# Triton-AI/Triton-Racer-Sim

Measured on AMD Instinct MI355X. Metric: env-steps/s (whole node) at N envs x 120x160 RGB, higher is better.
Workload: dtype f32 state / f64 nearest-point / u8 image; 1 GPU; 1024 envs/GPU x 1 GPU, bicycle physics + L1 nearest point + 120x160 RGB pinhole rasteriser = BASELINE configs[2], generated_track 1185 pts, synthetic controls seed 0x5EED, auto-reset; envs_total=1024, envs_per_gpu=1024, img_h=120, img_w=160, depth=False, steps_per_launch=1, step_mode=resident worker (posted steps), prewarm_steps=8400, launcher=self

## Files before the change

triton-racer-sim_amd/csrc/trsim_device.hpp:

```cpp
#pragma once
#include <hip/hip_runtime.h>

#include <cstdint>

#include "../../include/trsim.h"
#include "../../include/trsim_spec.h"
#include "trsim_plan.hpp"
#include "trsim_tables.hpp"

#ifndef TRS_ABLATE
#define TRS_ABLATE 0
#endif

namespace trsim {

struct PParams {
    float *x, *y, *z, *yaw, *v, *speed, *cte, *ep_return, *last_return, *steer_filt;
    int32_t *seg_idx, *ep_len;
    uint8_t *done, *pending;
    const float *ctl_steer, *ctl_thr, *ctl_brk;
    const uint8_t* ctl_reset;
    int ctl_stride;
    float4* cam;
    const unsigned char* blob;
    const float* start_yaw;
    const float* tangent_g;
    unsigned long long* stats;
    unsigned long long* fault;
    int n_envs, env_id_base, envs_per_wg, np;
    int off_py, off_pz, off_tan, blob_bytes, off_scratch, tan_in_lds;
    int off_gstart, off_gpts, grid_nx, grid_nz;
    double grid_x0, grid_z0;
    float map_x0f, map_z0f, inv_cellf;
    float dt, max_steer, inv_wheelbase, accel_max, drag_lin, roll_res, brake_max;
    float v_max, v_rev_max, offtrack_cte, offtrack_penalty, cam_fwd;
    int auto_reset, synth, n_steps, write_cam;
// ... 265 lines not shown
    best_out = __hiloint2double(__builtin_amdgcn_readlane(__double2hiint(best), 63), __builtin_amdgcn_readlane(__double2loint(best), 63));
}

__device__ __forceinline__ NearParams near_of(const PParams& p)
{
    return NearParams{p.np, p.off_py, p.off_pz, p.off_gstart, p.off_gpts, p.grid_nx, p.grid_nz, p.grid_x0, p.grid_z0};
}

struct EnvRegs {
    float x, y, z, yaw, v, sf, epr, speed, cte;
    int seg, epl, done, pend;
};

__device__ __forceinline__ void env_load(const PParams& p, int e, EnvRegs& s)
{
    s.pend = coherent_load(&p.pending[e]); s.done = coherent_load(&p.done[e]);
    s.sf = coherent_load(&p.steer_filt[e]);
    s.x = coherent_load(&p.x[e]); s.y = coherent_load(&p.y[e]); s.z = coherent_load(&p.z[e]);
    s.yaw = coherent_load(&p.yaw[e]); s.v = coherent_load(&p.v[e]);
    s.seg = coherent_load(&p.seg_idx[e]);
    s.epr = coherent_load(&p.ep_return[e]);
    s.epl = coherent_load(&p.ep_len[e]);
    s.speed = 0.f; s.cte = 0.f;
}

__device__ __forceinline__ void env_store(const PParams& p, int e, const EnvRegs& s, int lane)
{
    if (lane == 0) {
        p.x[e] = s.x; p.y[e] = s.y; p.z[e] = s.z; p.yaw[e] = s.yaw; p.v[e] = s.v;
        p.speed[e] = s.speed; p.cte[e] = s.cte; p.seg_idx[e] = s.seg; p.done[e] = (uint8_t)s.done;
        p.ep_return[e] = s.epr; p.ep_len[e] = s.epl; p.steer_filt[e] = s.sf; p.pending[e] = (uint8_t)s.pend;
    }
}
struct StepOut { float4 cam; float pitch; int is_done, do_reset; };

template <bool WT, typename T>
__device__ __forceinline__ void store_out(T* ptr, T v)
{
    if constexpr (WT) __hip_atomic_store(ptr, v, __ATOMIC_RELAXED, __HIP_MEMORY_SCOPE_SYSTEM);
    else *ptr = v;
}

template <bool WT, bool STORE_LR = true, bool SEL = false>
__device__ __forceinline__ void env_advance(const PParams& p, const unsigned char* lphys, int e, EnvRegs& s, uint32_t t, int synth,
                                            float steer, float thr, float brk, uint8_t rin, int lane, StepOut& o, const trsim::HillBlock* hill = nullptr)
{
    const double* lpx = reinterpret_cast<const double*>(lphys);
    const double* lpy = reinterpret_cast<const double*>(lphys + p.off_py);
    const double* lpz = reinterpret_cast<const double*>(lphys + p.off_pz);
    const float2* ltan = reinterpret_cast<const float2*>(lphys + p.off_tan);
    const int gid = p.env_id_base + e;
    float sf = s.sf;
    const int prev_idx = s.seg;
    float epr = s.epr;
    int epl = s.epl;
    const int do_reset = (s.pend != 0) || (rin != 0) || (p.auto_reset && s.done != 0);
    float x1, y0, z1, yaw1, v2, hs, hc;
    if (do_reset) {
        const int si = (int)(((long long)TRS_START_STRIDE * gid) % p.np);
        x1 = (float)lpx[si]; y0 = (float)lpy[si]; z1 = (float)lpz[si];
        yaw1 = p.start_yaw[si]; v2 = 0.0f; sf = 0.0f;
        if constexpr (SEL) spec_sincos_sel(yaw1, hs, hc); else spec_sincos(yaw1, hs, hc);
    } else {
        if (synth) synth_controls(p.seed, (uint32_t)gid, t, sf, steer, thr);
        steer = clampf(steer, -1.0f, 1.0f);
        thr = clampf(thr, -1.0f, 1.0f);
        brk = clampf(brk, 0.0f, 1.0f);
// ... 67 lines not shown
        const size_t ci = (size_t)k * (size_t)p.ctl_stride + (size_t)e;
        steer = p.ctl_steer[ci]; thr = p.ctl_thr[ci]; brk = p.ctl_brk ? p.ctl_brk[ci] : 0.0f;
    }
    StepOut o;
    env_advance<false, true, SEL>(p, lphys, e, s, t, p.synth, steer, thr, brk, rin, lane, o, hill);
    if (lane == 0) {
        if (p.write_cam) cam_out[e] = o.cam;
        *lcam_slot = o.cam;
        if (hill) {
            if (p.write_cam) hill->cam_pitch[(size_t)(t & (kRing - 1)) * p.n_envs + e] = o.pitch;
            if (lpitch_slot) *lpitch_slot = o.pitch;
        }
        if (o.is_done) atomicAdd(&p.stats[0], 1ull);
        if (o.do_reset) atomicAdd(&p.stats[1], 1ull);
        __hip_atomic_store(pprog_j, k + 1, __ATOMIC_RELEASE, __HIP_MEMORY_SCOPE_WORKGROUP);
    }
}

__device__ __forceinline__ f2v ray_step(f2v kk2, f2v cns)
{
#ifdef TRS_PACKED_RAY_STEP
    return kk2 * cns;
#else
    float dx, dz;
    asm("v_mul_f32 %0, %1, %2" : "=v"(dx) : "v"(kk2.x), "v"(cns.x));
    asm("v_mul_f32 %0, %1, %2" : "=v"(dz) : "v"(kk2.y), "v"(cns.y));
    return f2v{dx, dz};
#endif
}

struct RasterThread {
    const f2v* lrow;
    const float* lrowdepth;
    unsigned pal_off;
    f2v ufa, ufb, ufc, ufd;
    unsigned gwm1, ghm1, pitch;
    int cg, vstart, vground, col_off, row_bytes;
};

__device__ __forceinline__ RasterThread raster_thread(const RParams& p, const unsigned char* lds, int tid)
{
    RasterThread t;
    t.lrow = reinterpret_cast<const f2v*>(lds + p.off_rowtab);
    t.lrowdepth = reinterpret_cast<const float*>(lds + p.off_depth);
    t.pal_off = (unsigned)p.off_pal;
    const float half_w = (float)(p.W / 2);
    t.gwm1 = (unsigned)(p.map_w - 1); t.ghm1 = (unsigned)(p.map_h - 1);
    t.cg = tid % p.gpr;
    const int r0 = tid / p.gpr;
    const float uf0 = (float)(t.cg << 2) + 0.5f - half_w;
    t.ufa = f2v{uf0, uf0}; t.ufb = f2v{uf0 + 1.0f, uf0 + 1.0f}; t.ufc = f2v{uf0 + 2.0f, uf0 + 2.0f}; t.ufd = f2v{uf0 + 3.0f, uf0 + 3.0f};
    t.pitch = (unsigned)p.map_pitch_b;
    t.vstart = r0 < p.rows_per_pass ? r0 : p.H;
    t.vground = t.vstart;
    while (t.vground < p.uni_rows) t.vground += p.rows_per_pass;
    t.row_bytes = p.gpr * 12;
    t.col_off = t.cg * 12;
    return t;
}

struct FrameDesc { __amdgpu_buffer_rsrc_t rgb, dep; };

template <bool DEPTH>
__device__ __forceinline__ FrameDesc frame_desc(const RParams& p, uint8_t* img, float* dep, int e)
{
    FrameDesc f;
    f.rgb = __builtin_amdgcn_make_buffer_rsrc(img + (size_t)e * ((size_t)p.gpe * 12), 0, (int)((size_t)p.gpe * 12), 0x00020000);
    f.dep = f.rgb;
    if constexpr (DEPTH) f.dep = __builtin_amdgcn_make_buffer_rsrc(dep + (size_t)e * ((size_t)p.gpe * 4), 0, (int)((size_t)p.gpe * 16), 0x00020000);
    return f;
}

template <bool DEPTH>
__device__ __forceinline__ void raster_uniform_rows(const RParams& p, const RasterThread& t, const FrameDesc& f, int uni_rows = -1)
{
    const int nu = uni_rows < 0 ? p.uni_rows : uni_rows;
    for (int v = t.vstart; v < nu; v += p.rows_per_pass) {
        const uint32_t c = *(lds_u32p)(uintptr_t)(t.pal_off + ((unsigned)v << 4));
        const u3v px3 = {__builtin_amdgcn_perm(c, c, 0x04020100u), __builtin_amdgcn_perm(c, c, 0x05040201u), __builtin_amdgcn_perm(c, c, 0x06050402u)};
        __builtin_amdgcn_raw_buffer_store_b96(px3, f.rgb, t.col_off + v * t.row_bytes, 0, TRS_STORE_AUX);
        if constexpr (DEPTH) {
            const unsigned dz = __float_as_uint(t.lrowdepth[v]);
            const u4v d4 = {dz, dz, dz, dz};
            __builtin_amdgcn_raw_buffer_store_b128(d4, f.dep, (t.cg + v * p.gpr) * 16, 0, TRS_STORE_AUX);
        }
    }
}

template <bool DEPTH, bool UNI_CHECK = false>
__device__ __forceinline__ void raster_ground_rows(const RParams& p, const RasterThread& t, const FrameDesc& f, const float4 cam)
{
    const f2v sc = {cam.z, cam.w}, cns = {cam.w, -cam.z}, camxz = {cam.x, cam.y};
    f2v rt = t.lrow[t.vground < p.H ? t.vground : 0];
    for (int v = t.vground; v < p.H; v += p.rows_per_pass) {
        const int vn = v + p.rows_per_pass;
        const f2v rtn = t.lrow[vn < p.H ? vn : v];
        const unsigned pal_a = t.pal_off + ((unsigned)v << 4);
        const f2v lz2 = {rt.x, rt.x}, kk2 = {rt.y, rt.y};
        f2v a;
        if constexpr (UNI_CHECK) {
            a.x = __builtin_fmaf(rt.x, sc.x, camxz.x);
            a.y = __builtin_fmaf(rt.x, sc.y, camxz.y);
        } else {
            a = __builtin_elementwise_fma(lz2, sc, camxz);
        }
        const f2v d = ray_step(kk2, cns);
        auto shade = [&](f2v uf) -> uint32_t {
            const f2v g = __builtin_elementwise_fma(uf, d, a);
            const unsigned ix = min(cvt_u32_sat(g.x), t.gwm1);
            const unsigned iz = min(cvt_u32_sat(g.y), t.ghm1);
            const unsigned xoff = (ix >> 2) & ~3u;
            unsigned waddr, paddr;
            asm("v_mad_u32_u24 %0, %1, %2, %3" : "=v"(waddr) : "v"(iz), "s"(t.pitch), "v"(xoff));
            const uint32_t w = *(lds_u32p)(uintptr_t)waddr;
            const uint32_t cls = __builtin_amdgcn_ubfe(w, ix << 1, 2);
            asm("v_lshl_add_u32 %0, %1, 2, %2" : "=v"(paddr) : "v"(cls), "v"(pal_a));
            return *(lds_u32p)(uintptr_t)paddr;
        };
#if TRS_ABLATE == 2
        const uint32_t c0p = (uint32_t)v, c1p = c0p + 1, c2p = c0p + 2, c3p = c0p + 3; (void)shade;
#else
        uint32_t c0p, c1p, c2p, c3p;
        if (UNI_CHECK && rt.y == 0.0f) c0p = c1p = c2p = c3p = *(lds_u32p)(uintptr_t)pal_a;
        else { c0p = shade(t.ufa); c1p = shade(t.ufb); c2p = shade(t.ufc); c3p = shade(t.ufd); }
#endif
        const uint32_t w0 = __builtin_amdgcn_perm(c1p, c0p, 0x04020100u);
        const uint32_t w1 = __builtin_amdgcn_perm(c2p, c1p, 0x05040201u);
        const uint32_t w2 = __builtin_amdgcn_perm(c3p, c2p, 0x06050402u);
#if TRS_ABLATE == 1
        asm volatile("" :: "v"(w0), "v"(w1), "v"(w2)); (void)f;
#else
        const u3v px3 = {w0, w1, w2};
        __builtin_amdgcn_raw_buffer_store_b96(px3, f.rgb, t.col_off + v * t.row_bytes, 0, TRS_STORE_AUX);
        if constexpr (DEPTH) {
            const unsigned dz = __float_as_uint(t.lrowdepth[v]);
            const u4v d4 = {dz, dz, dz, dz};
            __builtin_amdgcn_raw_buffer_store_b128(d4, f.dep, (t.cg + v * p.gpr) * 16, 0, TRS_STORE_AUX);
        }
#endif
        rt = rtn;
    }
}


__device__ __forceinline__ uint32_t hill_filter_colour(const trsim::HillBlock& hb, uint32_t bgr)
{
    int t[3];
#pragma unroll
    for (int ch = 0; ch < 3; ++ch) {
        float x = (float)((bgr >> (8 * ch)) & 255u);
        x = x - hb.f_offset;
        x = x * hb.f_contrast;
        x = x + hb.f_offset;
        x = x < 0.0f ? 0.0f : (x > 255.0f ? 255.0f : x);
        t[ch] = (int)x;
    }
    int o0 = t[0], o1 = t[1], o2 = t[2];
    if (hb.f_color) {
        const int r = t[0], g = t[1], b = t[2];
        const int vv = max(r, max(g, b)), vmin = min(r, min(g, b)), diff = vv - vmin;
        const int sat = (diff * hb.hsv_tab[vv] + (1 << 11)) >> 12;
        int h = (vv == r) ? (g - b) : ((vv == g) ? (b - r + 2 * diff) : (r - g + 4 * diff));
        h = (h * hb.hsv_tab[256 + diff] + (1 << 11)) >> 12;
        if (h < 0) h += 180;
        const int hh = min(h, 255), ss = min(sat, 255);
#pragma unroll
        for (int f = 0; f < 4; ++f) {
            if (f >= hb.f_nfilters) break;
            const int lo = (int)hb.f_lo[f], hi = (int)hb.f_hi[f];
            const bool in = hh >= (lo & 255) && hh <= (hi & 255) && ss >= ((lo >> 8) & 255) && ss <= ((hi >> 8) & 255) && vv >= ((lo >> 16) & 255) && vv <= ((hi >> 16) & 255);
            const int val = in ? 255 : 0, d = hb.f_dst[f];
            o0 = d == 0 ? val : o0; o1 = d == 1 ? val : o1; o2 = d == 2 ? val : o2;
        }
    }
// ... 20 lines not shown
            if (lg) { c0 = trsim::light_colour(c0, lg); if (hb.filt) c0 = hill_filter_colour(hb, c0); c1 = c2 = c3 = c0; }
        } else {
            lz = zd * hb.inv_cell_f; kk = (t * hb.inv_f) * hb.inv_cell_f; dep = zd;
            const float fw = hb.fog_f * (zd * hb.inv_zfar_f), om = 1.0f - fw;
            constexpr int base[4][3] = {TRS_RGB_GRASS, TRS_RGB_ROAD, TRS_RGB_EDGE, TRS_RGB_CENTRE};
            constexpr int fog[3] = TRS_RGB_FOG;
            uint32_t col[4];
#pragma unroll
            for (int c = 0; c < 4; ++c) {
                uint32_t rgb = 0;
#pragma unroll
                for (int ch = 0; ch < 3; ++ch) {
                    const float a = (float)base[c][ch] * om, b = (float)fog[ch] * fw;
                    const float sum = a + b;
                    rgb |= (uint32_t)(int)(sum + 0.5f) << (8 * ch);
                }
                if (lg) rgb = trsim::light_colour(rgb, lg);
                col[c] = hb.filt ? hill_filter_colour(hb, rgb) : rgb;
            }
            c0 = col[0]; c1 = col[1]; c2 = col[2]; c3 = col[3];
        }
    }
    unsigned char* const tab = lds + tab_off;
    reinterpret_cast<f2v*>(tab)[v] = f2v{lz, kk};
    reinterpret_cast<u4v*>(tab + 8 * p.H)[v] = u4v{c0, c1, c2, c3};
    reinterpret_cast<float*>(tab + 24 * p.H)[v] = dep;
    return kk;
}

__device__ __forceinline__ RasterThread raster_use_table(const RasterThread& t, const unsigned char* lds, unsigned tab_off, int H)
{
    RasterThread r = t;
    r.lrow = reinterpret_cast<const f2v*>(lds + tab_off);
    r.pal_off = tab_off + 8u * (unsigned)H;
    r.lrowdepth = reinterpret_cast<const float*>(lds + tab_off + 24u * (unsigned)H);
    return r;
}

template <typename Bail>
__device__ __forceinline__ bool team_barrier_wait(const int* dbar, int target, Bail& bail)
{
    for (unsigned spins = 0; __hip_atomic_load(dbar, __ATOMIC_ACQUIRE, __HIP_MEMORY_SCOPE_WORKGROUP) < target; ++spins) {
        __builtin_amdgcn_s_sleep(1);
        if ((spins & 1023u) == 1023u && bail(spins == 1023u)) return false;
    }
    return true;
}

template <typename Bail>
__device__ __forceinline__ bool hill_batch_build(const RParams& p, unsigned char* lds, unsigned tab0, const float (&P)[kHillBatchMax], int nb, int* hbar, int done_before,
                                                 int tid, int lane, Bail& bail, const float* lg0 = nullptr)
{
    constexpr int nrw = kRasterThreads / 64;
    int* const fg = hbar + 4 + 4 * ((done_before / (2 * nrw)) & 1);
    if (tid < kHillBatchMax) fg[tid] = p.H;
    asm volatile("s_waitcnt lgkmcnt(0)" ::: "memory");
    if (lane == 0) __hip_atomic_fetch_add(hbar, 1, __ATOMIC_RELEASE, __HIP_MEMORY_SCOPE_WORKGROUP);
    if (!team_barrier_wait(hbar, done_before + nrw, bail)) return false;
    const unsigned tb = (unsigned)hill_table_bytes(p.H);
    for (int row = tid; row < nb * p.H; row += kRasterThreads) {
        const int bi = row / p.H, v = row - bi * p.H;
        const float Pv = bi == 0 ? P[0] : (bi == 1 ? P[1] : (bi == 2 ? P[2] : P[3]));
        if (hill_row_build(p, lds, tab0 + (unsigned)bi * tb, Pv, v, lg0 ? lg0 + 8 * bi : nullptr) != 0.0f) __hip_atomic_fetch_min(&fg[bi], v, __ATOMIC_RELAXED, __HIP_MEMORY_SCOPE_WORKGROUP);
    }
    asm volatile("s_waitcnt lgkmcnt(0)" ::: "memory");
    if (lane == 0) __hip_atomic_fetch_add(hbar, 1, __ATOMIC_RELEASE, __HIP_MEMORY_SCOPE_WORKGROUP);
    return team_barrier_wait(hbar, done_before + 2 * nrw, bail);
}

template <bool DEPTH>
__device__ __forceinline__ void raster_hill_frame(const RParams& p, const RasterThread& rth, const unsigned char* lds, unsigned tab0, int bi, const int* hbar, int done_before,
                                                  const FrameDesc& f, const float4 cam)
{
    constexpr int nrw = kRasterThreads / 64;
    const int first_ground = hbar[4 + 4 * ((done_before / (2 * nrw)) & 1) + bi];
    RasterThread t = raster_use_table(rth, lds, tab0 + (unsigned)(bi * hill_table_bytes(p.H)), p.H);
    raster_uniform_rows<DEPTH>(p, t, f, first_ground);
    int vg = t.vstart;
    if (vg < first_ground) vg += ((first_ground - vg + p.rows_per_pass - 1) / p.rows_per_pass) * p.rows_per_pass;
    t.vground = vg;
    raster_ground_rows<DEPTH, true>(p, t, f, cam);
}

__device__ __forceinline__ unsigned light_wave_palette(const RParams& p, unsigned pal0, const float* lg, int filt, int wave, int lane)
{
    const unsigned dst = pal0 + (unsigned)((wave % light_copies(p.gpr)) * p.H * 16);
    const int lo = (64 * wave) / p.gpr, hi = min((64 * wave + 63) / p.gpr, p.rows_per_pass - 1);
    const trsim::HillBlock& hb = *reinterpret_cast<const trsim::HillBlock*>(p.blob + trsim::hill_block_offset(p.blob_bytes));
    float gb[8];
#pragma unroll
    for (int k = 0; k < 8; ++k) gb[k] = lg[k];
    asm volatile("" ::: "memory");
    for (int r0 = lo; r0 <= hi; ++r0)
        for (int i = lane; r0 + (i >> 2) * p.rows_per_pass < p.H; i += 64) {
            const unsigned ent = ((unsigned)(r0 + (i >> 2) * p.rows_per_pass) << 4) + ((unsigned)(i & 3) << 2);
            uint32_t c = trsim::light_colour(*(lds_u32p)(uintptr_t)((unsigned)p.off_pal + ent), gb);
            if (filt) c = hill_filter_colour(hb, c);
            *(__attribute__((address_space(3))) uint32_t*)(uintptr_t)(dst + ent) = c;
        }
    asm volatile("" ::: "memory");
    return dst;
}

template <bool DEPTH, int NR>
struct LensCache {
    static constexpr int R = NR;
    float4 F[R], L[R], D[DEPTH ? R : 1];
    uint2 M[R];
};
template <bool DEPTH> using LensCacheStep = LensCache<DEPTH, DEPTH ? 3 : 8>;
template <bool DEPTH> using LensCacheWorker = LensCache<DEPTH, DEPTH ? 3 : 4>;

__device__ __forceinline__ int lens_col(const RParams& p, const RasterThread& t, bool& right)
{
// ... 439 lines not shown
```

triton-racer-sim_amd/csrc/trsim_hip.hip:

```cpp
#include <hip/hip_runtime.h>

#include <algorithm>
#include <array>
#include <cmath>
#include <cstdint>
#include <cstdio>
#include <cstring>
#include <string>
#include <utility>
#include <vector>

#include "../../include/trsim.h"
#include "../../include/trsim_spec.h"
#include "trsim_device.hpp"
#include "trsim_env.hpp"
#include "trsim_internal.hpp"
#include "trsim_tables.hpp"


#define TRS_EXPORT extern "C" __attribute__((visibility("default")))

namespace {


// ... 213 lines not shown
            if ((e - e_begin) % kDynBatch != 0) continue;
            const int nbatch = (e_end - e_begin + kDynBatch - 1) / kDynBatch;
            const int it = (sidx - sp.r_first) * nbatch + (e - e_begin) / kDynBatch;
            float4 cams[kDynBatch];
#pragma unroll
            for (int bi = 0; bi < kDynBatch; ++bi) {
                const int eb = e + bi;
                cams[bi] = make_float4(0.f, 0.f, 0.f, 1.f);
                if (eb < e_end) {
                    const int j = eb - e_begin;
                    if (sidx < 0) cams[bi] = lcam_prev[j];
                    else {
                        while (__hip_atomic_load(&pprog[j], __ATOMIC_ACQUIRE, __HIP_MEMORY_SCOPE_WORKGROUP) < sidx + 1) __builtin_amdgcn_s_sleep(2);
                        cams[bi] = lcam[sidx * sp.cam_stride + j];
                    }
                }
            }
            (void)raster_dyn_batch<DEPTH, LIGHT>(p, sp.fp, rth, smem, cams, min(kDynBatch, e_end - e), img, dep, e, it, tid, lane, [](bool) { return false; },
                                                 LIGHT ? llight + (e - e_begin) * 8 : nullptr, lds_off_lpal);
            continue;
        }
        const FrameDesc fd = frame_desc<DEPTH>(p, img, dep, e);
        RasterThread rl = rth;
        if constexpr (LIGHT && !HILLS && !DYN) rl.pal_off = light_wave_palette(p, lds_off_lpal, llight + (e - e_begin) * 8, lfilt, wave, lane);
        if (!((sp.skip_uniform >> (abs_step & 1u)) & 1)) raster_uniform_rows<DEPTH>(p, rl, fd);
        float4 cam;
        const int j = e - e_begin;
        if (sidx < 0) {
            cam = lcam_prev[j];
        } else {
            while (__hip_atomic_load(&pprog[j], __ATOMIC_ACQUIRE, __HIP_MEMORY_SCOPE_WORKGROUP) < sidx + 1) __builtin_amdgcn_s_sleep(2);
            cam = lcam[sidx * sp.cam_stride + j];
        }
        raster_ground_rows<DEPTH>(p, rl, fd, cam);
    }
    }
    STAMP(5);
}

using StepKernel = void (*)(SParams);
template <Variant V> StepKernel step_kernel_of()
{
    if constexpr (variant_built(V)) return &trs_step_kernel<(V & kVDepth) != 0, (V & kVDyn) != 0, (V & kVHills) != 0, (V & kVLens) != 0, (V & kVLight) != 0>;
    else return nullptr;
}
template <Variant... V> std::array<StepKernel, kVariants> step_kernel_table(std::integer_sequence<Variant, V...>) { return {step_kernel_of<V>()...}; }
const std::array<StepKernel, kVariants> kStepKernels = step_kernel_table(std::make_integer_sequence<Variant, kVariants>{});

#undef STAMP_STATS
struct PreParams {
    const uint8_t* src; uint8_t* dst;
    const int* hsv_tab;
    int n_img, H, W, gpr, gpe, r0, r1;
    int dynamic, color, n_filters;
    float contrast, offset;
    double baseline;
    unsigned lo[4], hi[4];
    int dst_ch[4];
    int edge, edge_low, edge_high, edge_ch;
    int off_mag, off_map, off_tab;
    unsigned char* scratch;
    size_t scratch_stride;
};

__device__ __forceinline__ u3v pack_rgb4(unsigned P0, unsigned P1, unsigned P2, unsigned P3)
{
    return u3v{__builtin_amdgcn_perm(P1, P0, 0x04020100u), __builtin_amdgcn_perm(P2, P1, 0x05040201u), __builtin_amdgcn_perm(P3, P2, 0x06050402u)};
// ... 2265 lines not shown
```

triton-racer-sim_amd/csrc/trsim_plan.hpp:

```cpp
#pragma once
#include <cstddef>
#include <string>
#include <vector>

#include "trsim_tables.hpp"

#ifndef TRS_RASTER_WAVES
#define TRS_RASTER_WAVES 8
#endif

namespace trsim {

constexpr int kRasterThreads = 64 * TRS_RASTER_WAVES;
constexpr int kPhysBlock = 256;
constexpr int kCamDepth = 4;
constexpr int kSlotWords = 20;
constexpr int kLensPalBytes = 513 * 16;
constexpr int kDynTabWords = 512 + 768 + 4 + 256;

using Variant = unsigned;
constexpr Variant kVDepth = 1, kVDyn = 2, kVHills = 4, kVLens = 8, kVLight = 16, kVariants = 32;
constexpr Variant variant_bits(bool depth, bool dyn, bool hills, bool lens, bool light)
{
    return (depth ? kVDepth : 0u) | (dyn ? kVDyn : 0u) | (hills ? kVHills : 0u) | (lens ? kVLens : 0u) | (light ? kVLight : 0u);
// ... 95 lines not shown
    int n = 0;
    while (n < 16 && step_lds_layout(lds_step, epw, H, W, v, n + 1).total <= 160 * 1024) ++n;
    return n;
}
inline bool resident_fits(int lds_step, int epw, int H, int W, Variant v) { return worker_lds_layout(lds_step, epw, H, W, v).total <= 160 * 1024; }
enum class LdsFit { ok, no_launch, no_worker };
inline LdsFit lds_fit(int lds_step, int epw, int H, int W, Variant v, bool resident)
{
    if (steps_that_fit(lds_step, epw, H, W, v) < 1) return LdsFit::no_launch;
    return resident && !resident_fits(lds_step, epw, H, W, v) ? LdsFit::no_worker : LdsFit::ok;
}

constexpr bool variant_keeps_uniform(Variant v) { return !(v & (kVDyn | kVLens | kVLight)); }
struct UniformRows {
    bool ok[2] = {false, false};
    void invalidate() { ok[0] = ok[1] = false; }
    unsigned skip_mask(Variant v) const { return variant_keeps_uniform(v) ? (ok[0] ? 1u : 0u) | (ok[1] ? 2u : 0u) : 0u; }
    void rendered(Variant v, unsigned long long first, unsigned long long n)
    {
        for (unsigned long long k = 0; k < n && k < 2; ++k) ok[(first + k) & 1ull] = variant_keeps_uniform(v);
    }
};

TRS_HD inline bool worker_skips_uniform(unsigned mask, unsigned long long start, unsigned long long s) { return ((mask >> (s & 1ull)) & 1u) != 0 || s - start >= 2; }
TRS_HD inline int worker_step_stores(int nstep, int nuni, bool skips) { return skips ? nstep - nuni : nstep; }
TRS_HD inline int worker_wait_count(unsigned mask, unsigned long long start, unsigned long long owed, unsigned long long s, int nstep, int nuni, int uni_now)
{
    int n = uni_now;
    for (unsigned long long q = owed + 1; q < s; ++q) n += worker_step_stores(nstep, nuni, worker_skips_uniform(mask, start, q));
    return n;
}
TRS_HD inline int worker_lag(int nstep, int nuni, bool skipping) { return (2 * worker_step_stores(nstep, nuni, skipping) + (skipping ? 0 : nuni) <= 63) ? 3 : 2; }

constexpr int kMaxLatencyTicks = 30;
struct ObsRing {
    int max_ticks = 0;
    bool on() const { return max_ticks > 0; }
    int slots() const { return max_ticks + 2; }
    int slot_of_step(long long T) const { const int S = slots(); return (int)(((T % S) + S) % S); }
    static bool arrived(long long T, int L) { return T - L >= 1; }
    int slot_of_obs(long long T, int L) const { return slot_of_step(T - (long long)L); }
    static int gather_buf(long long T) { return (int)(T & 1ll); }
};

struct TrackLayout {
    struct Phys { int off_py, off_pz, off_tan, tan_in_lds, off_gstart, off_gpts, blob_bytes, off_scratch, pts_bytes, lds_p; } p;
    struct Raster { int map_pitch_b, off_rowtab, off_pal, off_depth, off_sky, blob_bytes, lds_r; } r;
    int lds_off_phys, lds_step;
};
int track_layout(const TrackTables& T, int H, bool render, int envs_per_wg, TrackLayout& L, std::string& err);
void pack_track_images(const TrackTables& T, int H, const TrackLayout& L, std::vector<unsigned char>& phys, std::vector<unsigned char>& raster);

}
```

triton-racer-sim_amd/csrc/trsim_resident.hip:

```cpp
#include <hip/hip_runtime.h>

#include <algorithm>
#include <array>
#include <atomic>
#include <chrono>
#include <cstdint>
#include <cstdlib>
#include <cstddef>
#include <cstring>
#include <mutex>
#include <string>
#include <utility>

#include "../../include/trsim.h"
#include "../../include/trsim_spec.h"
#include "trsim_device.hpp"
#include "trsim_env.hpp"
#include "trsim_internal.hpp"

#define TRS_EXPORT extern "C" __attribute__((visibility("default")))

namespace trsim {

constexpr int kSlots = 8;
// ... 432 lines not shown
        const unsigned char* const lphys = smem + wp.lds_off_phys;
        u64 s = wp.start;
        for (;; ++s) {
            const int r = (int)(s - wp.start);
            if (!wait_posted(wp, l, D, s, lane)) break;
            const u64* en = reinterpret_cast<const u64*>(&wp.dc->ring[s & (kSlots - 1)]);
            const u64 ev = lane < 6 ? agent_load64(en + lane) : 0ull;
            const float* const c_st = reinterpret_cast<const float*>(lane_u64(ev, 1));
            const float* const c_th = reinterpret_cast<const float*>(lane_u64(ev, 2));
            const float* const c_br = reinterpret_cast<const float*>(lane_u64(ev, 3));
            const uint8_t* const c_rs = reinterpret_cast<const uint8_t*>(lane_u64(ev, 4));
            const int synth = (int)(unsigned)lane_u64(ev, 5);
            for (int j = pw - first; j < n_loc; j += nphys) {
                const int e = e_begin + j;
                if (r >= kCamDepth && !wait_lds_ge(wp, l, &D, &l.rread[j], (r - kCamDepth + 1) * (kRasterThreads / 64), 2u, lane)) return;
                float steer = 0.f, thr = 0.f, brk = 0.f;
                uint8_t rin = 0;
                if (!synth) {
                    steer = sys_load_val(&c_st[e]); thr = sys_load_val(&c_th[e]);
                    if (c_br) brk = sys_load_val(&c_br[e]);
                    if (c_rs) rin = sys_load_val(&c_rs[e]);
                }
                float* const q = l.lst + (size_t)j * 16;
                EnvRegs st;
                st.x = q[0]; st.y = q[1]; st.z = q[2]; st.yaw = q[3]; st.v = q[4]; st.sf = q[5]; st.epr = q[6];
                st.seg = __float_as_int(q[7]); st.epl = __float_as_int(q[8]); st.done = __float_as_int(q[9]); st.pend = __float_as_int(q[10]);
                st.speed = 0.f; st.cte = 0.f;
                float lr = q[11];
                const float epr_before = st.epr;
                StepOut o;
                if (n_loc <= TRS_PHYS_PRIO_MAX_ENVS) __builtin_amdgcn_s_setprio(3);
                env_advance<true, false>(P, lphys, e, st, (uint32_t)s, synth, steer, thr, brk, rin, lane, o,
                                         HILLS ? reinterpret_cast<const trsim::HillBlock*>(p.blob + trsim::hill_block_offset(p.blob_bytes)) : nullptr);
                if (n_loc <= TRS_PHYS_PRIO_MAX_ENVS) __builtin_amdgcn_s_setprio(0);
                if (o.do_reset) lr = epr_before;
                if constexpr (LIGHT) {
                    const float lv = lane < 8 ? sys_load_val(&light_g[(size_t)e * 8 + lane]) : 0.f;
                    if (lane < 8) lring[((size_t)(r & (kCamDepth - 1)) * epw + j) * 8 + lane] = lv;
                }
                if (lane == 0) {
                    q[0] = st.x; q[1] = st.y; q[2] = st.z; q[3] = st.yaw; q[4] = st.v; q[5] = st.sf; q[6] = st.epr;
                    q[7] = __int_as_float(st.seg); q[8] = __int_as_float(st.epl); q[9] = __int_as_float(st.done); q[10] = __int_as_float(st.pend);
                    q[11] = lr;
                    float* const sl = l.slot + ((size_t)(r & (kCamDepth - 1)) * epw + j) * kSlotWords;
                    *reinterpret_cast<float4*>(sl) = o.cam;
                    sl[4] = st.x; sl[5] = st.y; sl[6] = st.z; sl[7] = st.yaw; sl[8] = st.v; sl[9] = st.speed; sl[10] = st.cte;
                    sl[11] = __int_as_float(st.seg); sl[12] = st.epr; sl[13] = __int_as_float(st.epl); sl[14] = st.sf; sl[15] = lr;
                    sl[16] = __int_as_float(st.done);
                    if constexpr (HILLS) sl[17] = o.pitch;
                    if (o.is_done) atomicAdd(&P.stats[0], 1ull);
                    if (o.do_reset) atomicAdd(&P.stats[1], 1ull);
                    drain_lds();
                    lds_store32(&l.pprog[j], r + 1);
                }
            }
        }
        if (D.forwarder) {
            u64 t0 = 0;
            for (unsigned spins = 0; D.fwd < s; ++spins) {
                forward_arrivals(wp, l, D.fwd, lane);
                if (lds_load64(l.word) & kAbortBit) break;
                __builtin_amdgcn_s_sleep(2);
                if ((spins & 1023u) == 1023u) {
                    const u64 now = (u64)wall_clock64();
                    if (t0 == 0) t0 = now;
                    else if (now - t0 > wp.safety_ticks) { worker_abort(wp, l, 4u); break; }
                }
            }
        }
        return;
    }

    const RasterThread rth = raster_thread(p, smem, tid);
    trsim::LensBlock lb{};
    LensCacheWorker<DEPTH> lcache;
    if constexpr (LENS) {
        lb = *reinterpret_cast<const trsim::LensBlock*>(p.blob + trsim::lens_block_offset(p.blob_bytes));
        lens_cache_load(p, rth, lb, lcache);
    }
    int nu = 0, ng = 0;
    for (int v = rth.vstart; v < p.uni_rows; v += p.rows_per_pass) ++nu;
    for (int v = rth.vground; v < p.H; v += p.rows_per_pass) ++ng;
// ... 109 lines not shown
                    }
                }
                u64 t0_bar = 0;
                auto bail = [&](bool first) -> bool {
                    if (lds_load64(l.word) & kAbortBit) return true;
                    const u64 now = (u64)wall_clock64();
                    if (first) { t0_bar = now; return false; }
                    if (now - t0_bar > wp.safety_ticks) { worker_abort(wp, l, 5u); return true; }
                    return false;
                };
                const int done_before = (r * nbatch + b0 / HB) * 2 * (kRasterThreads / 64);
                if (!hill_batch_build(p, smem, (unsigned)wp.lds_off_hill, Pv, nb, hbar, done_before, tid, lane, bail,
                                      LIGHT ? lring + ((size_t)(r & (kCamDepth - 1)) * epw + b0) * 8 : nullptr)) return;
                if (LIGHT && lane == 0)
                    for (int bi = 0; bi < nb; ++bi) __hip_atomic_fetch_add(&l.rread[b0 + bi], 1, __ATOMIC_RELAXED, __HIP_MEMORY_SCOPE_WORKGROUP);
#pragma unroll
                for (int bi = 0; bi < kHillBatchMax; ++bi)
                    if (bi < nb)
                        raster_hill_frame<DEPTH>(p, rth, smem, (unsigned)wp.lds_off_hill, bi, hbar, done_before, frame_desc<DEPTH>(p, img, dep, e_begin + b0 + bi), cams[bi]);
                if (mine_j >= 0 && !(kDiag & 2)) {
                    const size_t e = (size_t)(e_begin + mine_j);
                    if (lane < 12) __hip_atomic_store((__attribute__((address_space(1))) unsigned*)(uintptr_t)optr + e, tel, __ATOMIC_RELAXED, __HIP_MEMORY_SCOPE_SYSTEM);
                    else if (lane < 14) __hip_atomic_store((__attribute__((address_space(1))) unsigned char*)(uintptr_t)optr + e, (unsigned char)(lane == 12 ? tel : 0u), __ATOMIC_RELAXED, __HIP_MEMORY_SCOPE_SYSTEM);
                }
            }
            continue;
        }
        if constexpr (LIGHT && !HILLS && !DYN) {
            for (int j = 0; j < n_loc; ++j) {
                const FrameDesc fd = frame_desc<DEPTH>(p, img, dep, e_begin + j);
                if (!wait_lds_ge(wp, l, nullptr, &l.pprog[j], r + 1, 3u, lane)) return;
                const float* const sl = l.slot + ((size_t)(r & (kCamDepth - 1)) * epw + j) * kSlotWords;
                const float4 cam = *reinterpret_cast<const float4*>(sl);
                const bool mine = (j % (kRasterThreads / 64)) == wave;
                unsigned tel = 0;
                if (mine) tel = __float_as_uint(sl[4 + min(lane, 12)]);
                RasterThread rl = rth;
                rl.pal_off = light_wave_palette(p, lds_off_lpal, lring + ((size_t)(r & (kCamDepth - 1)) * epw + j) * 8, lfilt, wave, lane);
                asm volatile("s_waitcnt lgkmcnt(0)" :: "v"(cam.x), "v"(cam.y), "v"(cam.z), "v"(cam.w), "v"(tel) : "memory");
                if (lane == 0) __hip_atomic_fetch_add(&l.rread[j], 1, __ATOMIC_RELAXED, __HIP_MEMORY_SCOPE_WORKGROUP);
                raster_uniform_rows<DEPTH>(p, rl, fd);
                if (j == 0)
                    while (s - owed >= keep) {
                        wait_vmcnt_le((int)(s - owed - 1) * nstep + nu);
                        raster_arrive(l, owed++, lane);
                    }
                raster_ground_rows<DEPTH>(p, rl, fd, cam);
                if (mine && !(kDiag & 2)) {
                    const size_t e = (size_t)(e_begin + j);
                    if (lane < 12) __hip_atomic_store((__attribute__((address_space(1))) unsigned*)(uintptr_t)optr + e, tel, __ATOMIC_RELAXED, __HIP_MEMORY_SCOPE_SYSTEM);
                    else if (lane < 14) __hip_atomic_store((__attribute__((address_space(1))) unsigned char*)(uintptr_t)optr + e, (unsigned char)(lane == 12 ? tel : 0u), __ATOMIC_RELAXED, __HIP_MEMORY_SCOPE_SYSTEM);
                }
            }
            continue;
        }
        const bool skipu = kSkipUniform && worker_skips_uniform(wp.uni_mask, wp.start, s);
        const bool sweep = ahead == 0 && !skipu;
        if (sweep)
            for (int j = 0; j < n_loc; ++j) raster_uniform_rows<DEPTH>(p, rth, frame_desc<DEPTH>(p, img, dep, e_begin + j));
        for (int j = 0; j < n_loc; ++j) {
            const FrameDesc fd = frame_desc<DEPTH>(p, img, dep, e_begin + j);
            if (!sweep && !skipu) raster_uniform_rows<DEPTH>(p, rth, fd);
            if (j == 0)
                while (s - owed >= keep) {
                    const u64 tv0 = probe ? now_clk() : 0;
                    if (!(kDiag & 1))
                        wait_vmcnt_le(kSkipUniform ? worker_wait_count(wp.uni_mask, wp.start, owed, s, nstep, nuni, skipu ? 0 : (sweep ? nuni : nu))
                                                   : (int)(s - owed - 1) * nstep + (sweep ? nuni : nu));
                    if (probe) t_vm += now_clk() - tv0;
                    raster_arrive(l, owed++, lane);
                }
            const u64 tq0 = probe ? now_clk() : 0;
            if (!wait_lds_ge(wp, l, nullptr, &l.pprog[j], r + 1, 3u, lane)) return;
            if (probe) t_pose += now_clk() - tq0;
            const float* const sl = l.slot + ((size_t)(r & (kCamDepth - 1)) * epw + j) * kSlotWords;
            const float4 cam = *reinterpret_cast<const float4*>(sl);
            const bool mine = (j % (kRasterThreads / 64)) == wave;
            unsigned tel = 0;
            if (mine) tel = __float_as_uint(sl[4 + min(lane, 12)]);
            asm volatile("s_waitcnt lgkmcnt(0)" :: "v"(cam.x), "v"(cam.y), "v"(cam.z), "v"(cam.w), "v"(tel) : "memory");
            if (lane == 0) __hip_atomic_fetch_add(&l.rread[j], 1, __ATOMIC_RELAXED, __HIP_MEMORY_SCOPE_WORKGROUP);
            if constexpr (LENS) raster_lens_frame(p, rth, lb, lcache, (unsigned)wp.lds_off_hill, fd, cam);
            else raster_ground_rows<DEPTH>(p, rth, fd, cam);
            if (mine && !(kDiag & 2)) {
                const size_t e = (size_t)(e_begin + j);
                if (lane < 12) __hip_atomic_store((__attribute__((address_space(1))) unsigned*)(uintptr_t)optr + e, tel, __ATOMIC_RELAXED, __HIP_MEMORY_SCOPE_SYSTEM);
                else if (lane < 14) __hip_atomic_store((__attribute__((address_space(1))) unsigned char*)(uintptr_t)optr + e, (unsigned char)(lane == 12 ? tel : 0u), __ATOMIC_RELAXED, __HIP_MEMORY_SCOPE_SYSTEM);
            }
        }
    }
}

using WorkerKernel = void (*)(WParams);
template <Variant V> WorkerKernel worker_kernel_of()
{
    if constexpr (variant_built(V)) return &trs_worker_kernel<(V & kVDepth) != 0, (V & kVDyn) != 0, (V & kVHills) != 0, (V & kVLens) != 0, (V & kVLight) != 0>;
    else return nullptr;
}
template <Variant... V> std::array<WorkerKernel, kVariants> worker_kernel_table(std::integer_sequence<Variant, V...>) { return {worker_kernel_of<V>()...}; }
const std::array<WorkerKernel, kVariants> kWorkerKernels = worker_kernel_table(std::make_integer_sequence<Variant, kVariants>{});

constexpr int kPwEnvs = 4;
constexpr int kPwBlock = 64 * (kPwEnvs + 2);

__global__ __launch_bounds__(kPwBlock) void trs_physics_worker_kernel(const WParams wp)
{
    const int tid = threadIdx.x, lane = tid & 63, wave = tid >> 6;
    const PParams& P = wp.ph;
    const WLds l = wlds_of(smem + wp.lds_off_ctl, kPwEnvs);
    const int e_begin = blockIdx.x * kPwEnvs;
    const int n_loc = min(e_begin + kPwEnvs, P.n_envs) - e_begin;
    if ((unsigned)(uintptr_t)smem != 0u) {
        if (tid == 0) {
            atomicAdd(&P.stats[2], 1ull);
            sys_store64(P.fault, 1ull);
            sys_store64(&wp.mb->error, (9ull << 32) | (u64)blockIdx.x);
// ... 604 lines not shown
```

Before: 125.1 million env-steps/s.

## Skip per-pixel map clamps on ground rows proven in-bounds by physics wave

The physics wave now computes, per env and per step, the first ground row from which every ray stays inside the ground map, by testing the two extreme columns of each row with a ballot. It passes that row index through the camera slot to the raster waves. Those waves render rows before it with the min clamps and the rest without them. The raster loop also switches from per-row index multiplies to incrementing LDS and buffer addresses. This trades two v_min per pixel for extra work on the physics wave and a wave-uniform loop split.

```diff
diff --git a/triton-racer-sim_amd/csrc/trsim_device.hpp b/triton-racer-sim_amd/csrc/trsim_device.hpp
--- a/triton-racer-sim_amd/csrc/trsim_device.hpp
+++ b/triton-racer-sim_amd/csrc/trsim_device.hpp
@@ -2,6 +2,7 @@
 #include <hip/hip_runtime.h>
 
 #include <cstdint>
+#include <type_traits>
 
 #include "../../include/trsim.h"
 #include "../../include/trsim_spec.h"
@@ -333,7 +334,7 @@
         p.ep_return[e] = s.epr; p.ep_len[e] = s.epl; p.steer_filt[e] = s.sf; p.pending[e] = (uint8_t)s.pend;
     }
 }
-struct StepOut { float4 cam; float pitch; int is_done, do_reset; };
+struct StepOut { float4 cam; float pitch; int is_done, do_reset; int vsafe; };
 
 template <bool WT, typename T>
 __device__ __forceinline__ void store_out(T* ptr, T v)
@@ -467,6 +468,7 @@
 struct RasterThread {
     const f2v* lrow;
     const float* lrowdepth;
+    unsigned row_off, dep_off;
     unsigned pal_off;
     f2v ufa, ufb, ufc, ufd;
     unsigned gwm1, ghm1, pitch;
@@ -478,6 +480,7 @@
     RasterThread t;
     t.lrow = reinterpret_cast<const f2v*>(lds + p.off_rowtab);
     t.lrowdepth = reinterpret_cast<const float*>(lds + p.off_depth);
+    t.row_off = (unsigned)p.off_rowtab; t.dep_off = (unsigned)p.off_depth;
     t.pal_off = (unsigned)p.off_pal;
     const float half_w = (float)(p.W / 2);
     t.gwm1 = (unsigned)(p.map_w - 1); t.ghm1 = (unsigned)(p.map_h - 1);
@@ -522,15 +525,45 @@
     }
 }
 
-template <bool DEPTH, bool UNI_CHECK = false>
-__device__ __forceinline__ void raster_ground_rows(const RParams& p, const RasterThread& t, const FrameDesc& f, const float4 cam)
-{
-    const f2v sc = {cam.z, cam.w}, cns = {cam.w, -cam.z}, camxz = {cam.x, cam.y};
-    f2v rt = t.lrow[t.vground < p.H ? t.vground : 0];
-    for (int v = t.vground; v < p.H; v += p.rows_per_pass) {
-        const int vn = v + p.rows_per_pass;
-        const f2v rtn = t.lrow[vn < p.H ? vn : v];
-        const unsigned pal_a = t.pal_off + ((unsigned)v << 4);
+typedef __attribute__((address_space(3))) const f2v* lds_f2vp;
+__device__ __forceinline__ int wave_first_safe_row(const RParams& p, const float4 cam, int lane)
+{
+    const float ufl = trsim::row_uf_left(p.W), ufr = trsim::row_uf_right(p.W);
+    const unsigned gwm1 = (unsigned)(p.map_w - 1), ghm1 = (unsigned)(p.map_h - 1);
+    int vsafe = p.uni_rows;
+    for (int v0 = p.uni_rows; v0 < p.H; v0 += 64) {
+        const int v = v0 + lane;
+        const f2v rt = *(lds_f2vp)(uintptr_t)((unsigned)p.off_rowtab + ((unsigned)min(v, p.H - 1) << 3));
+        const bool out = v < p.H && trsim::row_needs_clamp(rt.x, rt.y, cam.x, cam.y, cam.z, cam.w, ufl, ufr, gwm1, ghm1);
+        const unsigned long long m = __builtin_amdgcn_ballot_w64(out);
+        if (m) vsafe = v0 + 64 - __builtin_clzll(m);
+    }
+    return vsafe;
+}
+
+template <bool DEPTH, bool UNI_CHECK = false, bool SAFE = true>
+__device__ __forceinline__ void raster_ground_rows(const RParams& p, const RasterThread& t, const FrameDesc& f, const float4 cam, const int vsafe)
+{
+    float nsin = -cam.z;
+    asm volatile("" : "+v"(nsin));
+    const f2v sc = {cam.z, cam.w}, cns = {cam.w, nsin}, camxz = {cam.x, cam.y};
+    const unsigned r_end = t.row_off + ((unsigned)p.H << 3), r_last = r_end - 8u, r_step = (unsigned)p.rows_per_pass << 3;
+    const unsigned r_safe = t.row_off + ((unsigned)vsafe << 3);
+    const unsigned pal_step = (unsigned)p.rows_per_pass << 4;
+    unsigned ra = t.row_off + ((unsigned)t.vground << 3);
+    unsigned pal_a = t.pal_off + ((unsigned)t.vground << 4);
+    int voff = t.col_off + t.vground * t.row_bytes;
+    const int v_step = p.rows_per_pass * t.row_bytes;
+    [[maybe_unused]] unsigned dep_a = 0;
+    [[maybe_unused]] int dvoff = 0;
+    if constexpr (DEPTH) {
+        dep_a = t.dep_off + ((unsigned)t.vground << 2);
+        dvoff = (t.cg + t.vground * p.gpr) * 16;
+    }
+    f2v rt = *(lds_f2vp)(uintptr_t)min(ra, r_last);
+    auto row = [&](auto clamp) {
+        const unsigned rn = ra + r_step;
+        const f2v rtn = *(lds_f2vp)(uintptr_t)min(rn, r_last);
         const f2v lz2 = {rt.x, rt.x}, kk2 = {rt.y, rt.y};
         f2v a;
         if constexpr (UNI_CHECK) {
@@ -542,8 +575,8 @@
         const f2v d = ray_step(kk2, cns);
         auto shade = [&](f2v uf) -> uint32_t {
             const f2v g = __builtin_elementwise_fma(uf, d, a);
-            const unsigned ix = min(cvt_u32_sat(g.x), t.gwm1);
-            const unsigned iz = min(cvt_u32_sat(g.y), t.ghm1);
+            unsigned ix = cvt_u32_sat(g.x), iz = cvt_u32_sat(g.y);
+            if constexpr (decltype(clamp)::value) { ix = min(ix, t.gwm1); iz = min(iz, t.ghm1); }
             const unsigned xoff = (ix >> 2) & ~3u;
             unsigned waddr, paddr;
             asm("v_mad_u32_u24 %0, %1, %2, %3" : "=v"(waddr) : "v"(iz), "s"(t.pitch), "v"(xoff));
@@ -553,7 +586,7 @@
             return *(lds_u32p)(uintptr_t)paddr;
         };
 #if TRS_ABLATE == 2
-        const uint32_t c0p = (uint32_t)v, c1p = c0p + 1, c2p = c0p + 2, c3p = c0p + 3; (void)shade;
+        const uint32_t c0p = (ra - t.row_off) >> 3, c1p = c0p + 1, c2p = c0p + 2, c3p = c0p + 3; (void)shade;
 #else
         uint32_t c0p, c1p, c2p, c3p;
         if (UNI_CHECK && rt.y == 0.0f) c0p = c1p = c2p = c3p = *(lds_u32p)(uintptr_t)pal_a;
@@ -566,15 +599,25 @@
         asm volatile("" :: "v"(w0), "v"(w1), "v"(w2)); (void)f;
 #else
         const u3v px3 = {w0, w1, w2};
-        __builtin_amdgcn_raw_buffer_store_b96(px3, f.rgb, t.col_off + v * t.row_bytes, 0, TRS_STORE_AUX);
+        __builtin_amdgcn_raw_buffer_store_b96(px3, f.rgb, voff, 0, TRS_STORE_AUX);
         if constexpr (DEPTH) {
-            const unsigned dz = __float_as_uint(t.lrowdepth[v]);
+            const unsigned dz = __float_as_uint(*(__attribute__((address_space(3))) const float*)(uintptr_t)dep_a);
             const u4v d4 = {dz, dz, dz, dz};
-            __builtin_amdgcn_raw_buffer_store_b128(d4, f.dep, (t.cg + v * p.gpr) * 16, 0, TRS_STORE_AUX);
+            __builtin_amdgcn_raw_buffer_store_b128(d4, f.dep, dvoff, 0, TRS_STORE_AUX);
+            dep_a += (unsigned)p.rows_per_pass << 2; dvoff += p.rows_per_pass * p.gpr * 16;
         }
 #endif
-        rt = rtn;
-    }
+        rt = rtn; ra = rn; pal_a += pal_step; voff += v_step;
+    };
+    unsigned r_lim = r_end;
+    if constexpr (SAFE) {
+        r_lim = ra;
+        while (__builtin_amdgcn_ballot_w64(r_lim < r_safe) != 0ull) r_lim += r_step;
+        r_lim = min(r_lim, r_end);
+    }
+    while (ra < r_lim) row(std::true_type{});
+    if constexpr (SAFE)
+        while (ra < r_end) row(std::false_type{});
 }
 
 
@@ -661,6 +704,7 @@
 {
     RasterThread r = t;
     r.lrow = reinterpret_cast<const f2v*>(lds + tab_off);
+    r.row_off = tab_off; r.dep_off = tab_off + 24u * (unsigned)H;
     r.pal_off = tab_off + 8u * (unsigned)H;
     r.lrowdepth = reinterpret_cast<const float*>(lds + tab_off + 24u * (unsigned)H);
     return r;
@@ -708,7 +752,7 @@
     int vg = t.vstart;
     if (vg < first_ground) vg += ((first_ground - vg + p.rows_per_pass - 1) / p.rows_per_pass) * p.rows_per_pass;
     t.vground = vg;
-    raster_ground_rows<DEPTH, true>(p, t, f, cam);
+    raster_ground_rows<DEPTH, true, false>(p, t, f, cam, p.H);
 }
 
 __device__ __forceinline__ unsigned light_wave_palette(const RParams& p, unsigned pal0, const float* lg, int filt, int wave, int lane)
diff --git a/triton-racer-sim_amd/csrc/trsim_hip.hip b/triton-racer-sim_amd/csrc/trsim_hip.hip
--- a/triton-racer-sim_amd/csrc/trsim_hip.hip
+++ b/triton-racer-sim_amd/csrc/trsim_hip.hip
@@ -269,7 +269,7 @@
             while (__hip_atomic_load(&pprog[j], __ATOMIC_ACQUIRE, __HIP_MEMORY_SCOPE_WORKGROUP) < sidx + 1) __builtin_amdgcn_s_sleep(2);
             cam = lcam[sidx * sp.cam_stride + j];
         }
-        raster_ground_rows<DEPTH>(p, rl, fd, cam);
+        raster_ground_rows<DEPTH, false, false>(p, rl, fd, cam, p.H);
     }
     }
     STAMP(5);
diff --git a/triton-racer-sim_amd/csrc/trsim_plan.hpp b/triton-racer-sim_amd/csrc/trsim_plan.hpp
--- a/triton-racer-sim_amd/csrc/trsim_plan.hpp
+++ b/triton-racer-sim_amd/csrc/trsim_plan.hpp
@@ -151,6 +151,36 @@
 }
 TRS_HD inline int worker_lag(int nstep, int nuni, bool skipping) { return (2 * worker_step_stores(nstep, nuni, skipping) + (skipping ? 0 : nuni) <= 63) ? 3 : 2; }
 
+TRS_HD inline unsigned cvt_u32_sat_spec(float x)
+{
+#if defined(__HIP_DEVICE_COMPILE__)
+    unsigned r;
+    asm("v_cvt_u32_f32 %0, %1" : "=v"(r) : "v"(x));
+    return r;
+#else
+    if (!(x > 0.0f)) return 0u;
+    return x >= 4294967296.0f ? 0xFFFFFFFFu : (unsigned)x;
+#endif
+}
+TRS_HD inline float row_uf_left(int W) { return 0.5f - (float)(W / 2); }
+TRS_HD inline float row_uf_right(int W) { return ((float)(((W / 4) - 1) << 2) + 0.5f - (float)(W / 2)) + 3.0f; }
+TRS_HD inline bool row_needs_clamp(float lz, float kk, float camx, float camz, float s, float c, float ufl, float ufr, unsigned gwm1, unsigned ghm1)
+{
+    const float ax = __builtin_fmaf(lz, s, camx), az = __builtin_fmaf(lz, c, camz);
+    const float dx = kk * c, dz = kk * (-s);
+    const unsigned xl = cvt_u32_sat_spec(__builtin_fmaf(ufl, dx, ax)), xr = cvt_u32_sat_spec(__builtin_fmaf(ufr, dx, ax));
+    const unsigned zl = cvt_u32_sat_spec(__builtin_fmaf(ufl, dz, az)), zr = cvt_u32_sat_spec(__builtin_fmaf(ufr, dz, az));
+    return (xl > xr ? xl : xr) > gwm1 || (zl > zr ? zl : zr) > ghm1;
+}
+TRS_HD inline int first_safe_row(const float* rowtab, int uni_rows, int H, int W, float camx, float camz, float s, float c, unsigned gwm1, unsigned ghm1)
+{
+    const float ufl = row_uf_left(W), ufr = row_uf_right(W);
+    int vsafe = uni_rows;
+    for (int v = uni_rows; v < H; ++v)
+        if (row_needs_clamp(rowtab[2 * v], rowtab[2 * v + 1], camx, camz, s, c, ufl, ufr, gwm1, ghm1)) vsafe = v + 1;
+    return vsafe;
+}
+
 constexpr int kMaxLatencyTicks = 30;
 struct ObsRing {
     int max_ticks = 0;
diff --git a/triton-racer-sim_amd/csrc/trsim_resident.hip b/triton-racer-sim_amd/csrc/trsim_resident.hip
--- a/triton-racer-sim_amd/csrc/trsim_resident.hip
+++ b/triton-racer-sim_amd/csrc/trsim_resident.hip
@@ -488,6 +488,8 @@
                 if (n_loc <= TRS_PHYS_PRIO_MAX_ENVS) __builtin_amdgcn_s_setprio(3);
                 env_advance<true, false>(P, lphys, e, st, (uint32_t)s, synth, steer, thr, brk, rin, lane, o,
                                          HILLS ? reinterpret_cast<const trsim::HillBlock*>(p.blob + trsim::hill_block_offset(p.blob_bytes)) : nullptr);
+                if constexpr (!HILLS && !LENS && !DYN) o.vsafe = wave_first_safe_row(p, o.cam, lane);
+                else o.vsafe = p.H;
                 if (n_loc <= TRS_PHYS_PRIO_MAX_ENVS) __builtin_amdgcn_s_setprio(0);
                 if (o.do_reset) lr = epr_before;
                 if constexpr (LIGHT) {
@@ -504,6 +506,7 @@
                     sl[11] = __int_as_float(st.seg); sl[12] = st.epr; sl[13] = __int_as_float(st.epl); sl[14] = st.sf; sl[15] = lr;
                     sl[16] = __int_as_float(st.done);
                     if constexpr (HILLS) sl[17] = o.pitch;
+                    sl[18] = __int_as_float(o.vsafe);
                     if (o.is_done) atomicAdd(&P.stats[0], 1ull);
                     if (o.do_reset) atomicAdd(&P.stats[1], 1ull);
                     drain_lds();
@@ -679,12 +682,13 @@
                 if (!wait_lds_ge(wp, l, nullptr, &l.pprog[j], r + 1, 3u, lane)) return;
                 const float* const sl = l.slot + ((size_t)(r & (kCamDepth - 1)) * epw + j) * kSlotWords;
                 const float4 cam = *reinterpret_cast<const float4*>(sl);
+                const int vsafe_v = __float_as_int(sl[18]);
                 const bool mine = (j % (kRasterThreads / 64)) == wave;
                 unsigned tel = 0;
                 if (mine) tel = __float_as_uint(sl[4 + min(lane, 12)]);
                 RasterThread rl = rth;
                 rl.pal_off = light_wave_palette(p, lds_off_lpal, lring + ((size_t)(r & (kCamDepth - 1)) * epw + j) * 8, lfilt, wave, lane);
-                asm volatile("s_waitcnt lgkmcnt(0)" :: "v"(cam.x), "v"(cam.y), "v"(cam.z), "v"(cam.w), "v"(tel) : "memory");
+                asm volatile("s_waitcnt lgkmcnt(0)" :: "v"(cam.x), "v"(cam.y), "v"(cam.z), "v"(cam.w), "v"(tel), "v"(vsafe_v) : "memory");
                 if (lane == 0) __hip_atomic_fetch_add(&l.rread[j], 1, __ATOMIC_RELAXED, __HIP_MEMORY_SCOPE_WORKGROUP);
                 raster_uniform_rows<DEPTH>(p, rl, fd);
                 if (j == 0)
@@ -692,7 +696,7 @@
                         wait_vmcnt_le((int)(s - owed - 1) * nstep + nu);
                         raster_arrive(l, owed++, lane);
                     }
-                raster_ground_rows<DEPTH>(p, rl, fd, cam);
+                raster_ground_rows<DEPTH>(p, rl, fd, cam, __builtin_amdgcn_readfirstlane(vsafe_v));
                 if (mine && !(kDiag & 2)) {
                     const size_t e = (size_t)(e_begin + j);
                     if (lane < 12) __hip_atomic_store((__attribute__((address_space(1))) unsigned*)(uintptr_t)optr + e, tel, __ATOMIC_RELAXED, __HIP_MEMORY_SCOPE_SYSTEM);
@@ -722,13 +726,14 @@
             if (probe) t_pose += now_clk() - tq0;
             const float* const sl = l.slot + ((size_t)(r & (kCamDepth - 1)) * epw + j) * kSlotWords;
             const float4 cam = *reinterpret_cast<const float4*>(sl);
+            const int vsafe_v = __float_as_int(sl[18]);
             const bool mine = (j % (kRasterThreads / 64)) == wave;
             unsigned tel = 0;
             if (mine) tel = __float_as_uint(sl[4 + min(lane, 12)]);
-            asm volatile("s_waitcnt lgkmcnt(0)" :: "v"(cam.x), "v"(cam.y), "v"(cam.z), "v"(cam.w), "v"(tel) : "memory");
+            asm volatile("s_waitcnt lgkmcnt(0)" :: "v"(cam.x), "v"(cam.y), "v"(cam.z), "v"(cam.w), "v"(tel), "v"(vsafe_v) : "memory");
             if (lane == 0) __hip_atomic_fetch_add(&l.rread[j], 1, __ATOMIC_RELAXED, __HIP_MEMORY_SCOPE_WORKGROUP);
             if constexpr (LENS) raster_lens_frame(p, rth, lb, lcache, (unsigned)wp.lds_off_hill, fd, cam);
-            else raster_ground_rows<DEPTH>(p, rth, fd, cam);
+            else raster_ground_rows<DEPTH>(p, rth, fd, cam, __builtin_amdgcn_readfirstlane(vsafe_v));
             if (mine && !(kDiag & 2)) {
                 const size_t e = (size_t)(e_begin + j);
                 if (lane < 12) __hip_atomic_store((__attribute__((address_space(1))) unsigned*)(uintptr_t)optr + e, tel, __ATOMIC_RELAXED, __HIP_MEMORY_SCOPE_SYSTEM);
```

After: 126.5 million env-steps/s (median of 6 runs). 1.2% higher.
